# om-ai-lab/OmChat

Hardware: AMD Instinct MI355X
Metric: images/sec prefill + decode tokens/sec, OmChat-13B TP=1/8; p50 TTFT (higher is better)
Workload: dtype bf16

## Files before the change

omchat_amd/csrc/gemv.hip:

```cpp
#include "kernels.h"
#include "rowdot.h"
#include <type_traits>

namespace {

struct GemvP {
  const void* X; const void* W; void* Y; const void* bias; const void* resid;
  int ldx, ldw, ldy, ldr, b, N, K, out_f32, ksplit;
  const float* w_scale;
  int y_packed;
  const void* norm_w; float norm_eps;
  unsigned* dyn;
  void* y_pack;
  unsigned long long* dbg;
  const unsigned char* mx_s;
  const unsigned char* x12_top;
  const unsigned char* x12_cnt;
  const unsigned* x12_patch;
#if OMCHAT_EXPERIMENTS
  int xskew;
#endif
};
#if OMCHAT_EXPERIMENTS
#define OM_DBG_MIN(slot, cond) do { if (p.dbg && (cond) && threadIdx.x == 0) atomicMax(p.dbg + (slot), ~wall_clock64()); } while (0)
// ... 1035 lines not shown
      if constexpr (EPI == EPI_SWIGLU) {
        const float gt = rnd<T>(acc[r]), up = rnd<T>(acc[r + RR]);
        ((T*)p.Y)[n] = fromf<T>(rnd<T>(silu(gt)) * up);
      } else {
        const float y = acc[r] + e_bias[r];
        if (p.out_f32) ((float*)p.Y)[n] = y;
        else ((T*)p.Y)[n] = fromf<T>(y);
      }
    }
  }
  if constexpr (EPI == EPI_SWIGLU) { OM_DBG_MAX(5, blockIdx.x + 64 >= gridDim.x); OM_DBG_MAX(16 + (blockIdx.x & 7), blockIdx.x + 512 >= gridDim.x); }
  if constexpr (EPI == EPI_NONE) OM_DBG_MAX(9, (blockIdx.x & 7) == 0);
}

template <typename T, int EPI, int RR, int NCH, bool F8, int WAVES = 4>
__global__ __launch_bounds__(WAVES * 64) void gemv_rows_norm_kernel(GemvP p) { gemv_rows_norm_body<T, EPI, RR, NCH, F8 ? WF_E4M3 : WF_16, WAVES>(p); }
template <typename T, int EPI, int RR, int NCH, int WAVES = 4>
__global__ __launch_bounds__(WAVES * 64) void gemv_rows_norm_mx4_kernel(GemvP p) { gemv_rows_norm_body<T, EPI, RR, NCH, WF_MX4, WAVES>(p); }
template <typename T, int EPI, int RR, int NCH>
__global__ __launch_bounds__(256) void gemv_rows_norm_x12_kernel(GemvP p) { gemv_rows_norm_body<T, EPI, RR, NCH, WF_X12, 4>(p); }

template <typename T, int EPI, int NCH, int F8>
__device__ __forceinline__ void gemv_rows_norm_loop_body(const GemvP& p, int per_wg, unsigned skew) {
  typedef typename V8<T>::type v8;
  constexpr int R = EPI == EPI_SWIGLU ? 2 : 1;
  __shared__ __attribute__((aligned(16))) T xs[NCH * 512];
  __shared__ float red[4];
  const int lane = threadIdx.x & 63, wave = __builtin_amdgcn_readfirstlane(threadIdx.x >> 6);
  const int n_out = EPI == EPI_SWIGLU ? p.N / 2 : p.N;
  int o0 = blockIdx.x * per_wg, o1 = o0 + per_wg < n_out ? o0 + per_wg : n_out;
  if constexpr (EPI == EPI_SWIGLU) OM_DBG_MIN(4, blockIdx.x < 8);
  if (skew) {
    const int l = blockIdx.x & 7;
    int pre = 0;
    for (int i = 0; i < l; ++i) pre += per_wg + (int)((skew >> (4 * i)) & 15u) - 8;
    o0 = (blockIdx.x >> 3) * 8 * per_wg + pre;
    o1 = o0 + per_wg + (int)((skew >> (4 * l)) & 15u) - 8;
    o1 = o1 < n_out ? o1 : n_out;
  }
  typedef typename RwW<F8>::type wreg_t;
  auto row_of = [&](int n, int r) { return EPI == EPI_SWIGLU ? 32 * (n >> 4) + (n & 15) + r * 16 : n; };
  auto load_w = [&](wreg_t (&w)[R][NCH], int n) {
#pragma unroll
    for (int r = 0; r < R; ++r) {
      const size_t row = (size_t)row_of(n, r);
#pragma unroll
      for (int c = 0; c < NCH; ++c) {
        int k = c * 512 + lane * 8;
        k = k < p.K ? k : 0;
        w[r][c] = rw_ldw<T, F8>(p, row, k);
      }
    }
  };
  wreg_t wa[R][NCH], wb[R][NCH], wc[R][NCH];
  const int u0 = o0 + wave;
  if (u0 < o1) load_w(wa, u0);
  if (u0 + 4 < o1) load_w(wb, u0 + 4);
  if (u0 + 8 < o1) load_w(wc, u0 + 8);
  constexpr int MC = (NCH + 3) / 4;
  rw_u32x4 xq[MC], nq[MC];
#pragma unroll
  for (int i = 0; i < MC; ++i) {
    const int c = wave + 4 * i, k = c * 512 + lane * 8;
    const rw_u32x4 z = {0u, 0u, 0u, 0u};
    const bool ok = c < NCH && k < p.K;
    xq[i] = ok ? *reinterpret_cast<const rw_u32x4*>((const T*)p.X + k) : z;
    nq[i] = ok ? *reinterpret_cast<const rw_u32x4*>((const T*)p.norm_w + k) : z;
  }
  __builtin_amdgcn_sched_barrier(0);
  float ss = 0.f;
#pragma unroll
  for (int i = 0; i < MC; ++i) {
    const v8 xv = __builtin_bit_cast(v8, xq[i]);
#pragma unroll
    for (int j = 0; j < 8; ++j) { const float v = tof(xv[j]); ss += v * v; }
  }
#pragma unroll
  for (int o = 32; o > 0; o >>= 1) ss += __shfl_xor(ss, o, 64);
  if (lane == 0) red[wave] = ss;
  asm volatile("s_waitcnt lgkmcnt(0)" ::: "memory");
  __builtin_amdgcn_s_barrier();
  const float inv = rsqrtf((((red[0] + red[1]) + red[2]) + red[3]) / (float)p.K + p.norm_eps);
#pragma unroll
  for (int i = 0; i < MC; ++i) {
    const int c = wave + 4 * i;
    if (c < NCH) {
      const v8 xv = __builtin_bit_cast(v8, xq[i]), wv = __builtin_bit_cast(v8, nq[i]);
      v8 o;
#pragma unroll
      for (int j = 0; j < 8; ++j) o[j] = fromf<T>(tof(wv[j]) * rnd<T>(tof(xv[j]) * inv));
      *reinterpret_cast<v8*>(xs + c * 512 + lane * 8) = o;
    }
  }
  asm volatile("s_waitcnt lgkmcnt(0)" ::: "memory");
  __builtin_amdgcn_s_barrier();
  rw_u32x4 xr[NCH];
#pragma unroll
  for (int c = 0; c < NCH; ++c) xr[c] = *reinterpret_cast<const rw_u32x4*>(xs + c * 512 + lane * 8);
  __builtin_amdgcn_sched_barrier(0);
  auto finish = [&](wreg_t (&w)[R][NCH], int n) {
    float acc[R];
#pragma unroll
    for (int r = 0; r < R; ++r) {
      float a = 0.f;
#pragma unroll
      for (int c = 0; c < NCH; ++c) {
        a = rw_dotw<T, F8>(w[r][c], xr[c], a);
      }
#pragma unroll
      for (int o = 32; o > 0; o >>= 1) a += __shfl_xor(a, o, 64);
      if constexpr (F8 == WF_E4M3) a *= p.w_scale[row_of(n, r)];
      acc[r] = a;
    }
    if (lane == 0) {
      if constexpr (EPI == EPI_SWIGLU) {
        const float gt = rnd<T>(acc[0]), up = rnd<T>(acc[R - 1]);
        ((T*)p.Y)[n] = fromf<T>(rnd<T>(silu(gt)) * up);
      } else {
        const float y = acc[0] + (p.bias ? tof(((const T*)p.bias)[n]) : 0.f);
        if (p.out_f32) ((float*)p.Y)[n] = y;
        else ((T*)p.Y)[n] = fromf<T>(y);
      }
    }
  };
  for (int u = u0; u < o1; u += 12) {
    finish(wa, u);
    if (u + 12 < o1) load_w(wa, u + 12);
    if (u + 4 < o1) {
      finish(wb, u + 4);
      if (u + 16 < o1) load_w(wb, u + 16);
    }
    if (u + 8 < o1) {
      finish(wc, u + 8);
      if (u + 20 < o1) load_w(wc, u + 20);
    }
  }
  if constexpr (EPI == EPI_SWIGLU) {
    OM_DBG_MAX(5, (blockIdx.x & 7) == 0);
    OM_DBG_MAX(16 + (blockIdx.x & 7), true);
  }
}

template <typename T, int EPI, int NCH, bool F8>
__global__ __launch_bounds__(256) void gemv_rows_norm_loop_kernel(GemvP p, int per_wg, unsigned skew) {
  gemv_rows_norm_loop_body<T, EPI, NCH, F8 ? WF_E4M3 : WF_16>(p, per_wg, skew);
}
template <typename T, int EPI, int NCH>
__global__ __launch_bounds__(256) void gemv_rows_norm_loop_mx4_kernel(GemvP p, int per_wg, unsigned skew) {
  gemv_rows_norm_loop_body<T, EPI, NCH, WF_MX4>(p, per_wg, skew);
}

constexpr int DYN_CH = 2;
constexpr int DYN_POOLS = 64;
template <typename T, int EPI, int NCH, int F8>
__device__ __forceinline__ void gemv_rows_norm_dyn_body(const GemvP& p) {
  typedef typename V8<T>::type v8;
  constexpr int R = EPI == EPI_SWIGLU ? 2 : 1;
  __shared__ __attribute__((aligned(16))) T xs[NCH * 512];
  __shared__ float red[4];
  const int lane = threadIdx.x & 63, wave = __builtin_amdgcn_readfirstlane(threadIdx.x >> 6);
  const int n_out = EPI == EPI_SWIGLU ? p.N / 2 : p.N;
  const int n_chunks = (n_out + DYN_CH - 1) / DYN_CH, pool_sz = (n_chunks + DYN_POOLS - 1) / DYN_POOLS;
  typedef typename RwW<F8>::type wreg_t;
  auto row_of = [&](int n, int r) { return EPI == EPI_SWIGLU ? 32 * (n >> 4) + (n & 15) + r * 16 : n; };
  auto load_w = [&](wreg_t (&w)[R][NCH], int n) {
#pragma unroll
    for (int r = 0; r < R; ++r) {
      const size_t row = (size_t)row_of(n, r);
#pragma unroll
      for (int c = 0; c < NCH; ++c) {
        int k = c * 512 + lane * 8;
        k = k < p.K ? k : 0;
        w[r][c] = rw_ldw<T, F8>(p, row, k);
      }
    }
  };
  int pool = 0;
  const int g0 = blockIdx.x % DYN_POOLS;
  auto pool_count = [&](int g) { const int lo = g * pool_sz; return lo >= n_chunks ? 0 : (lo + pool_sz <= n_chunks ? pool_sz : n_chunks - lo); };
  auto ticket = [&]() -> unsigned {
    unsigned t = 0;
    if (lane == 0) t = __hip_atomic_fetch_add(p.dyn + 64 * ((g0 + pool) % DYN_POOLS), 1u, __ATOMIC_RELAXED, __HIP_MEMORY_SCOPE_AGENT);
    return t;
  };
  auto resolve = [&](unsigned t) -> int {
    int tk = (int)__builtin_amdgcn_readfirstlane(t);
    for (;;) {
      const int g = (g0 + pool) % DYN_POOLS;
      if (tk < pool_count(g)) return g * pool_sz + tk;
      if (++pool >= DYN_POOLS) return -1;
      tk = (int)__builtin_amdgcn_readfirstlane(ticket());
    }
  };
  int cur = resolve(ticket());
  unsigned nxt_t = cur >= 0 ? ticket() : 0u;
  wreg_t wa[R][NCH], wb[R][NCH], wc[R][NCH];
  auto out_ok = [&](int chunk, int i) { return chunk >= 0 && chunk * DYN_CH + i < n_out; };
  if (out_ok(cur, 0)) load_w(wa, cur * DYN_CH);
  if (out_ok(cur, 1)) load_w(wb, cur * DYN_CH + 1);
  constexpr int MC = (NCH + 3) / 4;
  rw_u32x4 xq[MC], nq[MC];
#pragma unroll
  for (int i = 0; i < MC; ++i) {
    const int c = wave + 4 * i, k = c * 512 + lane * 8;
    const rw_u32x4 z = {0u, 0u, 0u, 0u};
    const bool ok = c < NCH && k < p.K;
    xq[i] = ok ? *reinterpret_cast<const rw_u32x4*>((const T*)p.X + k) : z;
    nq[i] = ok ? *reinterpret_cast<const rw_u32x4*>((const T*)p.norm_w + k) : z;
  }
  __builtin_amdgcn_sched_barrier(0);
  float ss = 0.f;
#pragma unroll
  for (int i = 0; i < MC; ++i) {
    const v8 xv = __builtin_bit_cast(v8, xq[i]);
#pragma unroll
    for (int j = 0; j < 8; ++j) { const float v = tof(xv[j]); ss += v * v; }
  }
#pragma unroll
  for (int o = 32; o > 0; o >>= 1) ss += __shfl_xor(ss, o, 64);
  if (lane == 0) red[wave] = ss;
  asm volatile("s_waitcnt lgkmcnt(0)" ::: "memory");
  __builtin_amdgcn_s_barrier();
  const float inv = rsqrtf((((red[0] + red[1]) + red[2]) + red[3]) / (float)p.K + p.norm_eps);
#pragma unroll
  for (int i = 0; i < MC; ++i) {
    const int c = wave + 4 * i;
    if (c < NCH) {
      const v8 xv = __builtin_bit_cast(v8, xq[i]), wv = __builtin_bit_cast(v8, nq[i]);
      v8 o;
#pragma unroll
      for (int j = 0; j < 8; ++j) o[j] = fromf<T>(tof(wv[j]) * rnd<T>(tof(xv[j]) * inv));
      *reinterpret_cast<v8*>(xs + c * 512 + lane * 8) = o;
    }
  }
  asm volatile("s_waitcnt lgkmcnt(0)" ::: "memory");
  __builtin_amdgcn_s_barrier();
  rw_u32x4 xr[NCH];
#pragma unroll
  for (int c = 0; c < NCH; ++c) xr[c] = *reinterpret_cast<const rw_u32x4*>(xs + c * 512 + lane * 8);
  __builtin_amdgcn_sched_barrier(0);
  auto finish = [&](wreg_t (&w)[R][NCH], int n) {
    float acc[R];
#pragma unroll
    for (int r = 0; r < R; ++r) {
      float a = 0.f;
#pragma unroll
      for (int c = 0; c < NCH; ++c) {
        a = rw_dotw<T, F8>(w[r][c], xr[c], a);
      }
#pragma unroll
      for (int o = 32; o > 0; o >>= 1) a += __shfl_xor(a, o, 64);
      if constexpr (F8 == WF_E4M3) a *= p.w_scale[row_of(n, r)];
      acc[r] = a;
    }
    if (lane == 0) {
      if constexpr (EPI == EPI_SWIGLU) {
        const float gt = rnd<T>(acc[0]), up = rnd<T>(acc[R - 1]);
        ((T*)p.Y)[n] = fromf<T>(rnd<T>(silu(gt)) * up);
      } else {
        const float y = acc[0] + (p.bias ? tof(((const T*)p.bias)[n]) : 0.f);
        if (p.out_f32) ((float*)p.Y)[n] = y;
        else ((T*)p.Y)[n] = fromf<T>(y);
      }
    }
  };
  while (cur >= 0) {
    const int nxt = resolve(nxt_t);
    if (nxt >= 0) nxt_t = ticket();
    if (out_ok(nxt, 0)) load_w(wc, nxt * DYN_CH);
    finish(wa, cur * DYN_CH);
    if (out_ok(nxt, 1)) load_w(wa, nxt * DYN_CH + 1);
    if (out_ok(cur, 1)) finish(wb, cur * DYN_CH + 1);
    cur = nxt;
    if (cur < 0) break;
    const int nx2 = resolve(nxt_t);
    if (nx2 >= 0) nxt_t = ticket();
    if (out_ok(nx2, 0)) load_w(wb, nx2 * DYN_CH);
    finish(wc, cur * DYN_CH);
    if (out_ok(nx2, 1)) load_w(wc, nx2 * DYN_CH + 1);
    if (out_ok(cur, 1)) finish(wa, cur * DYN_CH + 1);
    cur = nx2;
    if (cur < 0) break;
    const int nx3 = resolve(nxt_t);
    if (nx3 >= 0) nxt_t = ticket();
    if (out_ok(nx3, 0)) load_w(wa, nx3 * DYN_CH);
    finish(wb, cur * DYN_CH);
    if (out_ok(nx3, 1)) load_w(wb, nx3 * DYN_CH + 1);
    if (out_ok(cur, 1)) finish(wc, cur * DYN_CH + 1);
    cur = nx3;
  }
  if (lane == 0) {
    const unsigned done = __hip_atomic_fetch_add(p.dyn + 64 * DYN_POOLS, 1u, __ATOMIC_RELAXED, __HIP_MEMORY_SCOPE_AGENT);
    if (done == gridDim.x * 4u - 1u) {
      for (int i = 0; i <= DYN_POOLS; ++i) __hip_atomic_store(p.dyn + 64 * i, 0u, __ATOMIC_RELAXED, __HIP_MEMORY_SCOPE_AGENT);
    }
  }
}

template <typename T, int EPI, int NCH, bool F8>
__global__ __launch_bounds__(256) void gemv_rows_norm_dyn_kernel(GemvP p) { gemv_rows_norm_dyn_body<T, EPI, NCH, F8 ? WF_E4M3 : WF_16>(p); }
template <typename T, int EPI, int NCH>
__global__ __launch_bounds__(256) void gemv_rows_norm_dyn_mx4_kernel(GemvP p) { gemv_rows_norm_dyn_body<T, EPI, NCH, WF_MX4>(p); }

template <typename T, int F8, int CP = 8, int G = 2>
__device__ __forceinline__ void gemv_rows_longk_body(const GemvP& p, int rows_per_wg) {
  static_assert(8 % CP == 0 && CP % G == 0, "whole passes cover ceil8(nch) chunks, whole decode groups a pass");
  extern __shared__ __attribute__((aligned(16))) char xs_raw[];
  T* xs = (T*)xs_raw;
  const int lane = threadIdx.x & 63, wave = __builtin_amdgcn_readfirstlane(threadIdx.x >> 6);
  const int nch = (p.K + 511) >> 9, npass8 = (nch + 7) >> 3, npass = npass8 * (8 / CP);
  const int n = blockIdx.x * rows_per_wg + wave;
  const bool valid = n < p.N;
  const int row = valid ? n : p.N - 1;
  OM_DBG_MIN(6, blockIdx.x < 8);
  typedef typename RwW<F8>::type wreg_t;
  auto load_w = [&](wreg_t (&w)[CP], int pass) {
#pragma unroll
    for (int c = 0; c < CP; ++c) {
      int k = (pass * CP + c) * 512 + lane * 8;
      k = k < p.K ? k : 0;
      if constexpr (F8 == WF_X12) w[c] = x12_ldw(p, (size_t)row, pass * CP + c < nch ? pass * CP + c : 0, pass * CP + c < nch ? lane : 0);
      else w[c] = rw_ldw<T, F8>(p, (size_t)row, k);
    }
  };
  float acc = 0.f;
  X12Row xst;
  auto dots = [&](wreg_t (&w)[CP], int pass) {
    if constexpr (F8 == WF_X12) {
#pragma unroll
      for (int h = 0; h < CP / G; ++h) {
        rw_u32x4 wd[G];
        x12_group<G>(wd, &w[G * h], xst, pass * CP + G * h, nch, lane);
#pragma unroll
        for (int c = 0; c < G; ++c) {
          const rw_u32x4 xr = *reinterpret_cast<const rw_u32x4*>(xs + (pass * CP + G * h + c) * 512 + lane * 8);
          acc = rw_dot8<T>(wd[c], xr, acc);
        }
      }
    } else {
#pragma unroll
      for (int c = 0; c < CP; ++c) {
        const rw_u32x4 xr = *reinterpret_cast<const rw_u32x4*>(xs + (pass * CP + c) * 512 + lane * 8);
        acc = rw_dotw<T, F8>(w[c], xr, acc);
      }
    }
  };
  wreg_t wa[CP], wb[CP], wc[CP];
  load_w(wa, 0);
  if constexpr (F8 == WF_X12) x12_row_load(xst, p, (size_t)row, lane);
  if (npass > 1) load_w(wb, 1);
  if (npass > 2) load_w(wc, 2);
  const float e_bias_raw = tof(((const T*)(p.bias ? p.bias : p.X))[p.bias ? row : 0]);
  const float e_res_raw = tof(((const T*)(p.resid ? p.resid : p.X))[p.resid ? row : 0]);
  const float e_bias = p.bias ? e_bias_raw : 0.f, e_res = p.resid ? e_res_raw : 0.f;
  float e_scale = 1.f;
  if constexpr (F8 == WF_E4M3) e_scale = p.w_scale[row];
  for (int i = threadIdx.x; i < npass8 * 8 * 64; i += blockDim.x) {
    const rw_u32x4 z = {0u, 0u, 0u, 0u};
    const rw_u32x4 v = i * 8 < p.K ? *reinterpret_cast<const rw_u32x4*>((const T*)p.X + i * 8) : z;
    *reinterpret_cast<rw_u32x4*>(xs + i * 8) = v;
  }
  __syncthreads();
  if constexpr (F8 == WF_X12) x12_row_finish(xst);
  for (int ps = 0; ps < npass; ps += 3) {
    if (ps > 0 && ps + 2 < npass) load_w(wc, ps + 2);
    dots(wa, ps);
    if (ps + 1 < npass) {
      if (ps + 3 < npass) load_w(wa, ps + 3);
      dots(wb, ps + 1);
    }
    if (ps + 2 < npass) {
      if (ps + 4 < npass) load_w(wb, ps + 4);
      dots(wc, ps + 2);
    }
  }
  float a = acc;
#pragma unroll
  for (int o = 32; o > 0; o >>= 1) a += __shfl_xor(a, o, 64);
  if constexpr (F8 == WF_E4M3) a *= e_scale;
  if (lane == 0 && valid) {
    const float y = rnd<T>(a + e_bias);
    ((T*)p.Y)[n] = fromf<T>(e_res + y);
  }
  OM_DBG_MAX(7, (blockIdx.x & 7) == 0);
}

template <typename T, bool F8>
__global__ __launch_bounds__(512) void gemv_rows_longk_kernel(GemvP p, int rows_per_wg) { gemv_rows_longk_body<T, F8 ? WF_E4M3 : WF_16>(p, rows_per_wg); }
template <typename T>
__global__ __launch_bounds__(512) void gemv_rows_longk_mx4_kernel(GemvP p, int rows_per_wg) { gemv_rows_longk_body<T, WF_MX4>(p, rows_per_wg); }
template <typename T>
__global__ __launch_bounds__(512) void gemv_rows_longk_x12_kernel(GemvP p, int rows_per_wg) { gemv_rows_longk_body<T, WF_X12, 4>(p, rows_per_wg); }

#if OMCHAT_EXPERIMENTS
template <typename T, int F8>
__device__ __forceinline__ void gemv_rows_longk_direct_body(const GemvP& p) {
  const int lane = threadIdx.x & 63, wave = __builtin_amdgcn_readfirstlane(threadIdx.x >> 6);
  const int nch = (p.K + 511) >> 9, npass = (nch + 7) >> 3;
  const int n = blockIdx.x * (int)(blockDim.x >> 6) + wave;
  if (n >= p.N) return;
  const int row = n;
  typedef typename RwW<F8>::type wreg_t;
  auto load_w = [&](wreg_t (&w)[8], int pass) {
#pragma unroll
    for (int c = 0; c < 8; ++c) {
      int k = (pass * 8 + c) * 512 + lane * 8;
      k = k < p.K ? k : 0;
      w[c] = rw_ldw<T, F8>(p, (size_t)row, k);
    }
  };
  auto load_x = [&](rw_u32x4 (&x)[8], int pass) {
#pragma unroll
    for (int c = 0; c < 8; ++c) {
      const int k = (pass * 8 + c) * 512 + lane * 8;
      const rw_u32x4 z = {0u, 0u, 0u, 0u};
      x[c] = k < p.K ? *reinterpret_cast<const rw_u32x4*>((const T*)p.X + k) : z;
    }
  };
  float acc = 0.f;
  auto dots = [&](wreg_t (&w)[8], rw_u32x4 (&x)[8]) {
#pragma unroll
    for (int c = 0; c < 8; ++c) {
      acc = rw_dotw<T, F8>(w[c], x[c], acc);
    }
  };
  wreg_t wa[8], wb[8];
  rw_u32x4 xa[8], xb[8];
  load_w(wa, 0);
  load_x(xa, 0);
  if (npass > 1) { load_w(wb, 1); load_x(xb, 1); }
  const float e_bias_raw = tof(((const T*)(p.bias ? p.bias : p.X))[p.bias ? row : 0]);
  const float e_res_raw = tof(((const T*)(p.resid ? p.resid : p.X))[p.resid ? row : 0]);
  const float e_bias = p.bias ? e_bias_raw : 0.f, e_res = p.resid ? e_res_raw : 0.f;
  float e_scale = 1.f;
  if constexpr (F8 == WF_E4M3) e_scale = p.w_scale[row];
  for (int ps = 0; ps < npass; ps += 2) {
    dots(wa, xa);
    if (ps + 2 < npass) { load_w(wa, ps + 2); load_x(xa, ps + 2); }
    if (ps + 1 < npass) {
      dots(wb, xb);
      if (ps + 3 < npass) { load_w(wb, ps + 3); load_x(xb, ps + 3); }
    }
  }
  float a = acc;
#pragma unroll
  for (int o = 32; o > 0; o >>= 1) a += __shfl_xor(a, o, 64);
  if constexpr (F8 == WF_E4M3) a *= e_scale;
  if (lane == 0) {
    const float y = rnd<T>(a + e_bias);
    ((T*)p.Y)[n] = fromf<T>(e_res + y);
  }
}

template <typename T, bool F8>
__global__ __launch_bounds__(256) void gemv_rows_longk_direct_kernel(GemvP p) { gemv_rows_longk_direct_body<T, F8 ? WF_E4M3 : WF_16>(p); }
template <typename T>
__global__ __launch_bounds__(256) void gemv_rows_longk_direct_mx4_kernel(GemvP p) { gemv_rows_longk_direct_body<T, WF_MX4>(p); }

#endif

int rows_per_wave(const GemvArgs& a, int wf, const GemvTuning& t, int n_cu) {
  if (a.norm_w) {
    if (wf == WF_X12) return a.epi == EPI_SWIGLU ? 1 : 4;
    if (a.epi == EPI_NONE) return a.N < 32768 ? 2 : 4;
    if (wf == WF_16) return t.gu_rr == 2 || t.gu_rr == 3 ? t.gu_rr : 1;
    return t.gu_rr8 == 2 || t.gu_rr8 == 1 ? t.gu_rr8 : 4;
  }
  if ((a.epi == EPI_NONE || a.epi == EPI_RESID) && a.N < 32768) return 1;
  if (wf != WF_16) return a.epi == EPI_NONE ? 8 : 4;
  return a.epi == EPI_SWIGLU && (t.shard & 4) && a.N / 2 < 16 * n_cu ? 1 : 4;
}
bool plan_balanced(GemvPlan& g, int n_out, int waves, const GemvTuning& t, int n_cu) {
  if (!t.rows_balance || n_out != waves * 2 * n_cu) return false;
  g.rr = 1; g.waves = waves; g.gx = 2 * n_cu; g.gy = 1; g.block = 64 * waves;
  return true;
}
void plan_rows(GemvPlan& g, const GemvArgs& a, int ks, const GemvTuning& t, int n_cu) {
  const int n_out = a.epi == EPI_SWIGLU ? a.N / 2 : a.N;
  g.family = GF_ROWS; g.waves = 4; g.block = 256; g.gy = ks;
  if (g.rr == 1 && a.epi == EPI_RESID && ks == 1 && plan_balanced(g, n_out, 7, t, n_cu)) return;
  g.gx = std::min(2048, cdiv(cdiv(n_out, g.rr), 4));
}
void plan_rows_norm(GemvPlan& g, const GemvArgs& a, const GemvTuning& t, int n_cu) {
  const int n_out = a.epi == EPI_SWIGLU ? a.N / 2 : a.N;
  const int chunks = cdiv(a.K, 512);
  g.family = GF_ROWS_NORM; g.waves = 4; g.block = 256; g.nch = chunks >= 1 && chunks <= 7 ? chunks : 8;
  if (g.wf != WF_X12 && g.nch >= 4) {
    const bool want = a.epi == EPI_SWIGLU ? (t.norm_loop & (g.wf != WF_16 ? 4 : 1)) : (a.N < 32768 ? (t.norm_loop & 2) : (t.norm_loop & 8));
    if (want && n_out >= 8 * n_cu) {
      g.rr = g.waves = 0;
      if (OMCHAT_EXPERIMENTS && a.dyn_ctr && t.dyn) { g.family = GF_ROWS_NORM_DYN; g.gx = 2 * n_cu; return; }
      g.family = GF_ROWS_NORM_LOOP;
      g.per_wg = cdiv(n_out, 2 * n_cu);
      g.skew = (t.skew >= 256u && n_out == g.per_wg * 2 * n_cu && (2 * n_cu) % 8 == 0) ? t.skew : 0u;
      g.gx = cdiv(n_out, g.per_wg);
      return;
    }
    if (a.epi == EPI_NONE && g.rr <= 2 && plan_balanced(g, n_out, 9, t, n_cu)) return;
  }
  g.gx = cdiv(cdiv(n_out, g.rr), 4);
  if (OMCHAT_EXPERIMENTS && g.wf != WF_X12 && a.epi == EPI_SWIGLU && g.rr == 1) {
    const int nwg = cdiv(n_out, 4), xs = (int)(t.skew < 256u ? t.skew : 0u);
    if (xs > 0 && nwg % 8 == 0 && n_out % 4 == 0 && xs < nwg / 8) { g.xskew = xs; g.gx = 8 * (nwg / 8 + xs); }
  }
}
void plan_longk(GemvPlan& g, const GemvArgs& a, const GemvTuning& t, int n_cu) {
  if (OMCHAT_EXPERIMENTS && t.longk_direct > 0) {
    g.family = GF_ROWS_LONGK_DIRECT; g.waves = std::min(4, t.longk_direct);
    if (g.wf == WF_X12) g.wf = WF_16;
    g.gx = cdiv(a.N, g.waves); g.block = 64 * g.waves;
    return;
  }
  g.family = GF_ROWS_LONGK;
  g.rows_per_wg = std::max(1, std::min(8, cdiv(a.N, 2 * n_cu)));
  g.gx = cdiv(a.N, g.rows_per_wg); g.block = 64 * g.rows_per_wg;
  g.lds = (cdiv(a.K, 512) + 7) / 8 * 8 * 512 * 2;
}
bool plan_xs(GemvPlan& g, const GemvArgs& a, int ks, const GemvTuning& t, int n_cu) {
  if (!a.w_packed || t.no_xs) return false;
  g.block = 512; g.nch = 7;
  const int tiles = a.N / 16, units = a.epi == EPI_SWIGLU ? a.N / 32 : tiles;
  if (OMCHAT_EXPERIMENTS && ks == 1 && (a.K >> 6) == 56 && a.epi == EPI_RESID) {
    g.family = GF_XS; g.gx = tiles;
    return true;
  }
  if (ks == 1 && (a.K >> 6) == 56 && a.N % 32 == 0 && (a.epi == EPI_SWIGLU || a.epi == EPI_NONE) &&
      (units >= 4 * n_cu || (a.epi == EPI_NONE && tiles >= n_cu && tiles <= 2 * n_cu) ||
       ((t.shard & 1) && a.epi == EPI_NONE && tiles < n_cu) || ((t.shard & 8) && a.epi == EPI_SWIGLU && units <= n_cu))) {
    g.family = GF_XS; g.norm = OMCHAT_EXPERIMENTS && a.epi == EPI_SWIGLU && a.norm_w;
    g.gx = units >= 4 * n_cu ? n_cu : (a.epi == EPI_SWIGLU || tiles < n_cu ? units : a.N / 32);
    return true;
  }
  if (a.epi == EPI_PARTIAL && ks > 1 && (a.K >> 6) % 8 == 0 && a.N % 16 == 0) {
    const int q = (a.K >> 6) / 8;
    int a5 = -1;
    for (int i = 0; i <= ks; ++i) if (5 * i + 2 * (ks - i) == q) a5 = i;
    int gx = std::max(1, n_cu / ks);
    if (tiles < 4 * gx && tiles % 2 == 0 && (long)tiles * ks >= n_cu && (long)tiles * ks <= 2L * n_cu) gx = tiles / 2;
    if (a5 >= 0 && (tiles >= 4 * gx || gx == tiles / 2)) {
      g.family = GF_XS_SPLIT; g.nch = 0; g.gx = gx; g.gy = ks; g.n5 = a5;
      return true;
    }
  }
  g.block = g.nch = 0;
  return false;
}
}

#define OM_NEED(cond, text) do { if (!(cond)) { g.refusal = text; return g; } } while (0)
GemvPlan gemv_plan(int dtype, const GemvArgs& a, const GemvTuning& t, int n_cu) {
  GemvPlan g{};
  OM_NEED(a.b >= 1 && a.b <= 32, "launch_gemv: batch must be 1..32 per call");
  OM_NEED(!a.x_packed || !a.w_scale, "launch_gemv: packed x: 16-bit or MXFP4 weights");
  OM_NEED(!(a.x_packed && a.mx_scale) || (a.w_packed && a.K % 64 == 0), "launch_gemv: packed x with MXFP4 weights: the packed MXFP4 replica (w_packed), K % 64 == 0");
  OM_NEED(!(a.w_scale && a.mx_scale), "launch_gemv: one weight format per launch: e4m3 (w_scale) or MXFP4 (mx_scale)");
  OM_NEED(!a.w_packed || (a.x_packed && a.N % 16 == 0), "launch_gemv: packed W needs packed x and N % 16 == 0");
  OM_NEED(!a.y_packed || (a.x_packed && a.epi == EPI_SWIGLU), "launch_gemv: packed y: SwiGLU epilogue of the packed kernel only");
  if (a.mx_scale) OM_NEED(a.K % 32 == 0 && a.ldw % 4 == 0 && a.ldx % 8 == 0, "launch_gemv: MXFP4 weights: K % 32 == 0 (one e8m0 scale per 32 k), ldw (bytes) % 4, ldx % 8");
  else OM_NEED(a.K % 64 == 0 && a.ldw % 8 == 0 && a.ldx % 8 == 0, "launch_gemv: K % 64, ldw % 8, ldx % 8");
  OM_NEED((!a.w_scale && !(a.mx_scale && !a.x_packed)) || a.b == 1, "launch_gemv: fp8 / MXFP4 weights: batch 1 only (MXFP4 at b > 1: packed x and the packed MXFP4 replica)");
  OM_NEED(a.epi == EPI_NONE || a.epi == EPI_RESID || a.epi == EPI_SWIGLU || a.epi == EPI_PARTIAL, "launch_gemv: bad epilogue");
  OM_NEED(a.ksplit <= 1 || a.epi == EPI_PARTIAL, "launch_gemv: ksplit > 1 only with EPI_PARTIAL (fp32 slices)");
  OM_NEED(a.ksplit <= (a.K + 63) / 64, "launch_gemv: ksplit exceeds the number of 64-wide K chunks");
  OM_NEED(a.epi != EPI_RESID || a.resid, "launch_gemv: resid missing");
  OM_NEED(a.epi != EPI_SWIGLU || a.N % 32 == 0, "launch_gemv: SwiGLU needs N % 32 == 0");
  OM_NEED(!(a.out_f32 && a.epi != EPI_NONE), "launch_gemv: fp32 output only with EPI_NONE");
  OM_NEED(dtype == OMCHAT_F16 || dtype == OMCHAT_BF16, "launch_gemv: bad dtype");
  const int ks = a.ksplit > 1 ? a.ksplit : 1;
  const bool mfma = a.force_mfma || t.force_mfma;
  g.epi = a.epi; g.gy = 1;
  g.wf = a.x12_top ? WF_X12 : a.mx_scale ? WF_MX4 : a.w_scale ? WF_E4M3 : WF_16;
  OM_NEED(!(a.norm_w && a.x_packed) || (a.w_packed && ks == 1 && (a.K >> 6) == 56 && a.epi == EPI_SWIGLU && a.N % 32 == 0 && !t.no_xs),
          "launch_gemv: the in-register RMSNorm on packed x exists for the x-stationary gate|up form only (packed W, K = 3584, no split-K)");
  OM_NEED(!(a.epi == EPI_RESID && a.x_packed) || (a.w_packed && ks == 1 && (a.K >> 6) == 56 && a.N % 16 == 0 && a.N / 16 <= n_cu && !t.no_xs),
          "launch_gemv: the batched residual epilogue exists for the x-stationary form only (packed W, K = 3584, N / 16 <= CUs, no split-K)");
  if (a.x_packed) {
    g.nb = a.b > 16 ? 2 : 1;
    if (g.wf == WF_X12) g.wf = WF_16;
    OM_NEED(!(a.mx_scale && (a.norm_w || a.epi == EPI_RESID)), "launch_gemv: the batched norm-in-GEMV / residual forms read 16-bit weights only (no MXFP4 instantiation)");
    OM_NEED(OMCHAT_EXPERIMENTS || !(a.norm_w || a.epi == EPI_RESID), "launch_gemv: the batched norm-in-GEMV / residual forms need a -DOMCHAT_EXPERIMENTS=1 build");
    if (plan_xs(g, a, ks, t, n_cu)) return g;
    OM_NEED(!a.norm_w, "launch_gemv: packed-x RMSNorm form: gate|up shape outside the x-stationary launch (N / 32 >= 4 CUs)");
    g.family = GF_PK; g.wpack = a.w_packed != 0; g.ntile = 2; g.waves = 8; g.unroll = 4;
    if (a.epi == EPI_PARTIAL) {
      const int cps = cdiv(a.K >> 6, ks);
      if ((t.shard & 2) && cps <= 32) { g.ntile = 1; g.unroll = cps <= 8 ? 1 : 2; }
      else if (a.K / ks >= 1536) { g.ntile = 4; g.waves = 4; g.unroll = 2; }
    } else if (a.epi == EPI_NONE && a.N >= 32768) { g.ntile = 4; g.waves = 4; }
    g.gx = cdiv(cdiv(a.N, 16), g.ntile); g.gy = ks; g.block = 64 * g.waves;
    return g;
  }
  if (a.x12_top) {
    const bool ok = dtype == OMCHAT_BF16 && a.b == 1 && !a.w_packed && ks == 1 && a.K >= 512 && a.K % 512 == 0 &&
                    a.ldw == a.K / 2 * 3 && a.x12_cnt && a.x12_patch && !a.w_scale && !a.mx_scale && !mfma;
    const bool norm = ok && a.norm_w && (a.epi == EPI_SWIGLU || a.epi == EPI_NONE) && a.K <= RW_MAXC * 512;
    const bool longk = ok && !a.norm_w && a.epi == EPI_RESID && !a.out_f32 && a.K > RW_MAXC * 512 && a.K <= 32768;
    OM_NEED(norm || longk, "launch_gemv: bf16x12 weights: bf16, b == 1, K % 512 == 0, and norm_w with EPI_SWIGLU / EPI_NONE (K <= 4096) or EPI_RESID on 4096 < K <= 32768");
    if (longk) plan_longk(g, a, t, n_cu);
    else { g.rr = rows_per_wave(a, WF_X12, t, n_cu); plan_rows_norm(g, a, t, n_cu); }
    return g;
  }
  if (a.b == 1 && a.epi == EPI_RESID && ks == 1 && !a.out_f32 && a.K > RW_MAXC * 512 && a.K % 8 == 0 && a.K <= 32768 && (!mfma || a.mx_scale)) {
    plan_longk(g, a, t, n_cu);
    return g;
  }
  const bool rows_ok = a.b == 1 && cdiv(cdiv(a.K, 512), ks) <= RW_MAXC;
  OM_NEED(!a.norm_w || (rows_ok && ks == 1 && !mfma && (a.epi == EPI_NONE || a.epi == EPI_SWIGLU)),
          "launch_gemv: the in-register RMSNorm needs the whole-row batch-1 form without split-K (K <= 4096), epilogue NONE / SWIGLU");
  OM_NEED(!(a.w_scale || a.mx_scale) || rows_ok, "launch_gemv: fp8 / MXFP4 weights need b == 1 and <= 8 chunks of 512 per K slice");
  if (rows_ok && (a.w_scale || a.mx_scale || !mfma)) {
    g.rr = rows_per_wave(a, g.wf, t, n_cu);
    if (a.norm_w) plan_rows_norm(g, a, t, n_cu);
    else plan_rows(g, a, ks, t, n_cu);
    return g;
  }
  g.family = GF_MFMA; g.nb = a.b > 16 ? 2 : 1; g.waves = 8; g.unroll = 4;
  g.ntile = a.epi == EPI_SWIGLU || (a.epi == EPI_NONE && (g.nb == 2 || a.N >= 16384)) ? 2 : 1;
  if (g.nb == 1 && a.epi == EPI_PARTIAL && a.K / 64 / ks <= 32) { g.waves = 4; g.unroll = 8; }
  if (g.nb == 1 && a.epi == EPI_NONE) g.unroll = 8;
  g.gx = cdiv(a.N, 16 * g.ntile); g.gy = ks; g.block = 64 * g.waves;
  return g;
}
#undef OM_NEED

int gemv_split_k(int b, int K, int H, bool packed, bool down, const GemvTuning& t) {
  if (b == 1) { const int nch = cdiv(K, 512); return nch >= 16 ? std::min(DEC_KS_MAX, nch) : std::max(1, std::min(3, nch)); }
  if (!down && packed && K == 3584) return 2;
  if ((t.shard & 2) && K / 64 <= 64) return std::max(1, std::min(DEC_KS_MAX, (K / 64) / 16));
  return std::max(1, std::min(DEC_KS_MAX, std::min(K / 64, (down ? 3 : 1) * cdiv(512, cdiv(H, 16)))));
}

namespace {
template <auto KERNEL, typename... A>
int launch_k(const GemvPlan& g, hipStream_t s, const A&... args) {
  hipLaunchKernelGGL(KERNEL, dim3(g.gx, g.gy), dim3(g.block), (size_t)g.lds, s, args...);
  return 0;
}
template <auto KERNEL, typename... A>
int launch_k_lds64(const GemvPlan& g, hipStream_t s, const A&... args) {
  static PerDeviceOnce set;
  if (set.first()) OM_HIP(hipFuncSetAttribute((const void*)KERNEL, hipFuncAttributeMaxDynamicSharedMemorySize, 64 * 1024));
  return launch_k<KERNEL>(g, s, args...);
}
template <int... V, typename F>
int with_int(int v, F&& f) {
  int rc = -1;
  (void)((v == V ? (rc = f(std::integral_constant<int, V>{}), true) : false) || ...);
  return rc;
}
#define IV(c) decltype(c)::value
constexpr bool rows_rr(int epi, int rr, bool q) {
  return epi == EPI_NONE ? rr == 1 || rr == (q ? 8 : 4) : epi == EPI_RESID ? rr == 1 || rr == 4 : epi == EPI_SWIGLU ? rr == 4 || (rr == 1 && !q) : rr == 4;
}
constexpr bool norm_rr(int epi, int rr, bool q) { return epi == EPI_NONE ? rr == 2 || rr == 4 : q ? rr == 1 || rr == 2 || rr == 4 : rr <= 3; }

template <typename T>
int gemv_launch(const GemvPlan& g, const GemvP& p, hipStream_t s) {
  switch (g.family) {
    case GF_MFMA:
#define OM_MFMA(NT_, EPI_, WV_, UN_, NB_)                                                                  \
  if (g.ntile == NT_ && g.epi == EPI_ && g.waves == WV_ && g.unroll == UN_ && g.nb == NB_)                 \
    return launch_k<gemv_kernel<T, NT_, EPI_, WV_, UN_, false, NB_>>(g, s, p)
      OM_MFMA(1, EPI_PARTIAL, 8, 4, 2); OM_MFMA(2, EPI_SWIGLU, 8, 4, 2); OM_MFMA(1, EPI_RESID, 8, 4, 2); OM_MFMA(2, EPI_NONE, 8, 4, 2);
      OM_MFMA(1, EPI_PARTIAL, 4, 8, 1); OM_MFMA(1, EPI_PARTIAL, 8, 4, 1); OM_MFMA(2, EPI_SWIGLU, 8, 4, 1); OM_MFMA(1, EPI_RESID, 8, 4, 1);
      OM_MFMA(2, EPI_NONE, 8, 8, 1); OM_MFMA(1, EPI_NONE, 8, 8, 1);
#undef OM_MFMA
      return -1;
    case GF_PK:
#define OM_PK(NT_, EPI_, WV_, UN_)                                                                         \
  if (g.ntile == NT_ && g.epi == EPI_ && g.waves == WV_ && g.unroll == UN_)                                \
    return with_int<1, 2>(g.nb, [&](auto NB) {                                                             \
      if (g.wf == WF_MX4) return launch_k<gemv_pk_mx4_kernel<T, NT_, EPI_, WV_, UN_, IV(NB)>>(g, s, p);      \
      if (g.wpack) return launch_k<gemv_pk_kernel<T, NT_, EPI_, WV_, UN_, IV(NB), true>>(g, s, p);           \
      return launch_k<gemv_pk_kernel<T, NT_, EPI_, WV_, UN_, IV(NB), false>>(g, s, p);                       \
    })
      OM_PK(2, EPI_SWIGLU, 8, 4); OM_PK(1, EPI_PARTIAL, 8, 1); OM_PK(1, EPI_PARTIAL, 8, 2); OM_PK(4, EPI_PARTIAL, 4, 2); OM_PK(2, EPI_PARTIAL, 8, 4);
      OM_PK(4, EPI_NONE, 4, 4); OM_PK(2, EPI_NONE, 8, 4);
#undef OM_PK
      return -1;
    case GF_XS:
      return with_int<1, 2>(g.nb, [&](auto NB) {
#if OMCHAT_EXPERIMENTS
        if (g.epi == EPI_RESID) return launch_k<gemv_xs_kernel<T, EPI_RESID, IV(NB), 7>>(g, s, p);
        if (g.norm) return launch_k<gemv_xs_kernel<T, EPI_SWIGLU, IV(NB), 7, true>>(g, s, p);
#endif
        return with_int<EPI_SWIGLU, EPI_NONE>(g.epi, [&](auto EPI) {
          if (g.wf == WF_MX4) return launch_k<gemv_xs_mx4_kernel<T, IV(EPI), IV(NB), 7>>(g, s, p);
          return launch_k<gemv_xs_kernel<T, IV(EPI), IV(NB), 7>>(g, s, p);
        });
      });
    case GF_XS_SPLIT:
      return with_int<1, 2>(g.nb, [&](auto NB) {
        if (g.wf == WF_MX4) return launch_k<gemv_xs_split_mx4_kernel<T, IV(NB)>>(g, s, p, g.n5);
        return launch_k<gemv_xs_split_kernel<T, IV(NB)>>(g, s, p, g.n5);
      });
// ... 365 lines not shown
```

Measured before the change: 384.4.

## Add NB-deep weight prefetch ring and batched X staging to long-K x12 GEMV

Adds an optional path to the long-K row GEMV body with a rotating ring of NB weight register buffers and a steady-state loop that issues the next load after each dot pass. The X vector is staged into shared memory in batches of XB loads before their stores, and the first weight loads are issued ahead of that staging. Scheduling barriers keep the compiler from reordering these phases. Only the x12 kernel enables it (NB=3, CP=4). The intent is more memory-level parallelism and hiding global latency, at the cost of extra VGPRs from the larger register ring and X buffer.

```diff
diff --git a/omchat_amd/csrc/gemv.hip b/omchat_amd/csrc/gemv.hip
--- a/omchat_amd/csrc/gemv.hip
+++ b/omchat_amd/csrc/gemv.hip
@@ -1361,7 +1361,7 @@
 template <typename T, int EPI, int NCH>
 __global__ __launch_bounds__(256) void gemv_rows_norm_dyn_mx4_kernel(GemvP p) { gemv_rows_norm_dyn_body<T, EPI, NCH, WF_MX4>(p); }
 
-template <typename T, int F8, int CP = 8, int G = 2>
+template <typename T, int F8, int CP = 8, int G = 2, int NB = 0, int XB = 6>
 __device__ __forceinline__ void gemv_rows_longk_body(const GemvP& p, int rows_per_wg) {
   static_assert(8 % CP == 0 && CP % G == 0, "whole passes cover ceil8(nch) chunks, whole decode groups a pass");
   extern __shared__ __attribute__((aligned(16))) char xs_raw[];
@@ -1403,7 +1403,80 @@
         acc = rw_dotw<T, F8>(w[c], xr, acc);
       }
     }
+    if constexpr (NB > 0) asm volatile("" : "+v"(acc));
   };
+  if constexpr (NB > 0) {
+    const int nx = npass8 * 8 * 64, bd = (int)blockDim.x;
+    const rw_u32x4 z = {0u, 0u, 0u, 0u};
+    auto xi = [&](int base, int j) { const int i = base + (int)threadIdx.x + j * bd; return i < nx ? i : (int)threadIdx.x; };
+    rw_u32x4 xv[XB];
+#pragma unroll
+    for (int j = 0; j < XB; ++j) {
+      xv[j] = *reinterpret_cast<const rw_u32x4*>((const T*)p.X + (xi(0, j) * 8 < p.K ? xi(0, j) * 8 : 0));
+    }
+    __builtin_amdgcn_sched_barrier(0);
+    wreg_t w[NB][CP];
+    load_w(w[0], 0);
+    if constexpr (F8 == WF_X12) x12_row_load(xst, p, (size_t)row, lane);
+    __builtin_amdgcn_sched_barrier(0);
+#pragma unroll
+    for (int b = 1; b < NB; ++b) {
+      if (b < 16 / CP || b < npass) load_w(w[b], b);
+    }
+    const float e_bias_raw = tof(((const T*)(p.bias ? p.bias : p.X))[p.bias ? row : 0]);
+    const float e_res_raw = tof(((const T*)(p.resid ? p.resid : p.X))[p.resid ? row : 0]);
+    const float e_bias = p.bias ? e_bias_raw : 0.f, e_res = p.resid ? e_res_raw : 0.f;
+    float e_scale = 1.f;
+    if constexpr (F8 == WF_E4M3) e_scale = p.w_scale[row];
+#pragma unroll
+    for (int j = 0; j < XB; ++j) {
+      *reinterpret_cast<rw_u32x4*>(xs + xi(0, j) * 8) = xi(0, j) * 8 < p.K ? xv[j] : z;
+    }
+    for (int base = XB * bd; base < nx; base += XB * bd) {
+#pragma unroll
+      for (int j = 0; j < XB; ++j) {
+        xv[j] = *reinterpret_cast<const rw_u32x4*>((const T*)p.X + (xi(base, j) * 8 < p.K ? xi(base, j) * 8 : 0));
+      }
+#pragma unroll
+      for (int j = 0; j < XB; ++j) {
+        *reinterpret_cast<rw_u32x4*>(xs + xi(base, j) * 8) = xi(base, j) * 8 < p.K ? xv[j] : z;
+      }
+    }
+    __syncthreads();
+    if constexpr (F8 == WF_X12) x12_row_finish(xst);
+    auto last = [&](int ps, auto rem) {
+#pragma unroll
+      for (int b = 0; b < decltype(rem)::value; ++b) {
+        dots(w[b % NB], ps + b);
+        if (b + NB < decltype(rem)::value) load_w(w[b % NB], ps + b + NB);
+      }
+    };
+    int ps = 0;
+#pragma unroll 1
+    for (; ps + 2 * NB <= npass; ps += NB) {
+#pragma unroll
+      for (int b = 0; b < NB; ++b) { dots(w[b], ps + b); load_w(w[b], ps + b + NB); }
+    }
+    switch (npass - ps) {
+      case 1: last(ps, std::integral_constant<int, 1>()); break;
+      case 2: last(ps, std::integral_constant<int, 2>()); break;
+      case 3: last(ps, std::integral_constant<int, 3 < 2 * NB ? 3 : 1>()); break;
+      case 4: last(ps, std::integral_constant<int, 4 < 2 * NB ? 4 : 1>()); break;
+      case 5: last(ps, std::integral_constant<int, 5 < 2 * NB ? 5 : 1>()); break;
+      case 6: last(ps, std::integral_constant<int, 6 < 2 * NB ? 6 : 1>()); break;
+      default: last(ps, std::integral_constant<int, 7 < 2 * NB ? 7 : 1>()); break;
+    }
+    float a = acc;
+#pragma unroll
+    for (int o = 32; o > 0; o >>= 1) a += __shfl_xor(a, o, 64);
+    if constexpr (F8 == WF_E4M3) a *= e_scale;
+    if (lane == 0 && valid) {
+      const float y = rnd<T>(a + e_bias);
+      ((T*)p.Y)[n] = fromf<T>(e_res + y);
+    }
+    OM_DBG_MAX(7, (blockIdx.x & 7) == 0);
+    return;
+  }
   wreg_t wa[CP], wb[CP], wc[CP];
   load_w(wa, 0);
   if constexpr (F8 == WF_X12) x12_row_load(xst, p, (size_t)row, lane);
@@ -1449,7 +1522,7 @@
 template <typename T>
 __global__ __launch_bounds__(512) void gemv_rows_longk_mx4_kernel(GemvP p, int rows_per_wg) { gemv_rows_longk_body<T, WF_MX4>(p, rows_per_wg); }
 template <typename T>
-__global__ __launch_bounds__(512) void gemv_rows_longk_x12_kernel(GemvP p, int rows_per_wg) { gemv_rows_longk_body<T, WF_X12, 4>(p, rows_per_wg); }
+__global__ __launch_bounds__(512) void gemv_rows_longk_x12_kernel(GemvP p, int rows_per_wg) { gemv_rows_longk_body<T, WF_X12, 4, 2, 3>(p, rows_per_wg); }
 
 #if OMCHAT_EXPERIMENTS
 template <typename T, int F8>
```

Measured after the change: 389.3 (median of 6 runs). +1.3%, better.
